# chao1224/MoleculeSDE

Hardware: AMD Instinct MI355X
Metric: molecules/sec pretrain step (SchNet+SDE VE, bs256) (higher is better)
Workload: dtype f32; 1 GPU; PCQM4Mv2-shaped pretrain step: GIN5x300 + SchNet(6x128f,51g,rc10) + EBM_node_dot_prod contrastive + SDEModel2Dto3D_02 VE; fwd+bwd+Adam; molecules_per_gpu=256, global_batch=256, parallelism=dp1

## Files before the change

### include/msde_hip.h

```cpp
#ifndef MSDE_HIP_H
#define MSDE_HIP_H

#ifdef __cplusplus
extern "C" {
#endif

#define MSDE_EINVAL (-1)
#define MSDE_EUNSUP (-2)

int msde_abi_version(void);
const char* msde_target_arch(void);

int msde_radius_count(const float* pos, const int* batch, const int* mol_ptr, int N, float r2,
                      int max_nbr, int* deg, void* stream);
int msde_exclusive_scan_i32(const int* in, int* out, int n, void* stream);
int msde_radius_fill(const float* pos, const int* batch, const int* mol_ptr, int N, float r2,
                     int max_nbr, const int* rowptr, int* src, int* dst, float* dist, int E_cap,
                     void* stream);


int msde_plan_build(const int* x_raw, int K, const int* atom_off, const int* bond_src, const int* bond_dst,
                    const int* bond_attr, const int* bond_off, const int* mol_atoms, const int* mol_bonds,
                    int B, int N_cap, int Eb_cap, int Ee_cap, int P_cap, int Er_cap, int max_nbr, int* mol_ptr,
                    int* bond_ptr, int* pair_ptr, int* sizes, int* batch_i32, int* atom_codes, int* z_codes, int* b_rowptr,
// ... 29 lines not shown
int msde_dd_transpose3(const float* x, int E, int to_soa, float* y, void* stream);
int msde_dd_merge3(const float* a, const float* b, const float* c, int E, float* y, void* stream);
int msde_dd_broadcast_rows(const float* b, int M, int K, float* y, void* stream);

int msde_combine_losses(const float* a, const float* b, const float* c, const float* d, float ca, float cb, float cc,
                        float cd, float* out, void* stream);
int msde_combine_losses_bwd(const float* g, float ca, float cb, float cc, float cd, float* out4, void* stream);
int msde_combine_losses_ex(const float* a, const float* b, const float* c, const float* d, float ca, float cb, float cc,
                           float cd, float* out, float* seeds4, const float* const* log_src, float* const* log_dst,
                           int n_log, void* stream);

int msde_debug_stamp(long long* slot, void* stream);

int msde_segment_sum_rows(const float* rows, int ldi ,
                          const int* rowptr, const int* perm, int N, int D,
                          float scale_by_inv_count, float* out, int ldo ,
                          void* stream);
int msde_segment_sum_rows2(const float* rows, int ldi, const int* rowptr, const int* perm, const int* rowptr2,
                           const int* perm2, int N, int D, float scale_by_inv_count, float* out, int ldo,
                           void* stream);
int msde_pair_gather_add(const float* A, const float* B, int ld, const int* src, const int* dst, int E,
                         int D, float* out, void* stream);
int msde_pair_gather_add_stats(const float* A, const float* B, int ld, const int* src, const int* dst, int E, int D,
                               const int* e_valid, float* out, float* stats, void* stream);
int msde_segment_sum_rows_bn(const float* G, const float* Z, int ld, const int* rowptr, const int* perm, int N, int D,
                             const float* p, const float* w, const float* u, float* out, int ldo, void* stream);
int msde_pair_strip(void);
int msde_pair_bn_dgrad_stats(const float* g, int ldg, const float* W, const float* Z, const float* scale, const float* shift,
                             const float* mean, int E, int H, int D, const int* e_valid, float* GA, float* stats,
                             void* stream);
int msde_pair_bn_scatter(const float* GA, const float* AB, int D, const int* src, const int* dst, const int* rowptr_s,
                         const int* perm_s, const int* rowptr, int N, const float* p, const float* w, const float* u,
                         float* gAB, void* stream);
int msde_pair_gather_cat(const float* X, int ldx, const float* C, int ldc, const int* src, const int* dst, int E,
                         int D, int D2, float* out, void* stream);
int msde_gather_rows(const float* X, const int* idx, int E, int D, float* out, void* stream);

int msde_radius_transpose(const int* batch, const int* mol_ptr, const int* rowptr, const int* src, int N,
                          int E_cap, int* deg_s, int* rowptr_s, int* perm_s, void* stream);
int msde_radius_transpose_mol(const int* mol_ptr, int B, int n_max, const int* rowptr, const int* src, int N, int E_cap,
                              int* rowptr_s, int* perm_s, void* stream);

int msde_embedding_sum_fwd(const float* tab, const int* codes, int N, int K, int D, float* out,
                           void* stream);
long long msde_embedding_sum_bwd_workspace_floats(int R, int D, int split);
int msde_embedding_sum_bwd(const float* g, const int* list_ptr, const int* list_nodes, int R,
                           int D, int split, float* g_tab, float* workspace, void* stream);

int msde_gin_aggregate_fwd(const float* x, const float* tab, const int* codes, const float* eps,
                           const int* rowptr, const int* src, int N, int D, float* out,
                           void* stream);
int msde_gin_aggregate_bwd_x(const float* g, const float* x, const float* tab, const int* codes,
                             const float* eps, const int* rowptr_s, const int* perm_s,
                             const int* dst, int N, int D, float* g_x, void* stream);
long long msde_gin_aggregate_bwd_tab_workspace_floats(int N, int E, int D, int R);
int msde_gin_aggregate_bn_fwd(const float* z, const float* scale, const float* shift, int relu, const float* tab,
                              const int* codes, const float* eps, const int* rowptr, const int* src, int N, int D,
                              float* h_out, float* out, void* stream);
int msde_gin_aggregate_bwd_x_stats(const float* g, const float* x, const float* tab, const int* codes, const float* eps,
                                   const int* rowptr_s, const int* perm_s, const int* dst, int N, const int* m_valid,
                                   int D, const float* zprev, const float* mean, int relu, float* g_x, float* stats,
                                   void* stream);
int msde_gin_aggregate_bwd_tab_slabs(int N, int E);
int msde_gin_aggregate_bwd_tab(const float* g, const float* x, const float* tab, const int* codes,
                               const int* src, const int* dst, int N, int E, int D, int R,
                               float* g_tab, float* g_eps, float* workspace, const int* n_dev, const int* e_dev,
// ... 440 lines not shown
```

### moleculesde_amd/_lib.py

```python
import ctypes
import os

_HERE = os.path.dirname(os.path.abspath(__file__))
LIB_PATH = os.path.join(_HERE, "csrc", "libmsde_hip.so")

P = ctypes.c_void_p
I = ctypes.c_int
F = ctypes.c_float
LL = ctypes.c_longlong
ULL = ctypes.c_ulonglong

SIGNATURES = {
    "msde_abi_version": [],
    "msde_target_arch": [],
    "msde_radius_count": [P, P, P, I, F, I, P, P],
    "msde_exclusive_scan_i32": [P, P, I, P],
    "msde_radius_fill": [P, P, P, I, F, I, P, P, P, P, I, P],
    "msde_segment_sum_rows": [P, I, P, P, I, I, F, P, I, P],
    "msde_segment_sum_rows2": [P, I, P, P, P, P, I, I, F, P, I, P],
    "msde_pair_gather_add": [P, P, I, P, P, I, I, P, P],
    "msde_pair_gather_add_stats": [P, P, I, P, P, I, I, P, P, P, P],
    "msde_segment_sum_rows_bn": [P, P, I, P, P, I, I, P, P, P, P, I, P],
    "msde_pair_strip": [],
    "msde_pair_bn_dgrad_stats": [P, I, P, P, P, P, P, I, I, I, P, P, P, P],
    "msde_pair_bn_scatter": [P, P, I, P, P, P, P, P, I, P, P, P, P, P],
    "msde_pair_gather_cat": [P, I, P, I, P, P, I, I, I, P, P],
    "msde_mlp_head_fwd": [P, I, P, P, I, I, I, P, P],
    "msde_mlp_head_bwd_slabs": [I, I],
    "msde_mlp_head_bwd": [P, I, P, P, I, I, I, P, P, P, P, P],
    "msde_mlp_head_mix_fwd": [P, I, P, P, I, P, P, I, P, P, P, P],
    "msde_mlp_head_mix_bwd": [P, I, P, P, P, P, P, I, I, P, P, P, P],
    "msde_gather_rows": [P, P, I, I, P, P],
    "msde_embedding_sum_fwd": [P, P, I, I, I, P, P],
    "msde_radius_transpose": [P, P, P, P, I, I, P, P, P, P],
    "msde_radius_transpose_mol": [P, I, I, P, P, I, I, P, P, P],
    "msde_embedding_sum_bwd_workspace_floats": [I, I, I],
    "msde_embedding_sum_bwd": [P, P, P, I, I, I, P, P, P],
    "msde_gin_aggregate_fwd": [P, P, P, P, P, P, I, I, P, P],
    "msde_gin_aggregate_bwd_x": [P, P, P, P, P, P, P, P, I, I, P, P],
    "msde_gin_aggregate_bn_fwd": [P, P, P, I, P, P, P, P, P, I, I, P, P, P],
    "msde_gin_aggregate_bwd_x_stats": [P, P, P, P, P, P, P, P, I, P, I, P, P, I, P, P, P],
    "msde_gin_aggregate_bwd_tab_workspace_floats": [I, I, I, I],
    "msde_gin_aggregate_bwd_tab": [P, P, P, P, P, P, I, I, I, I, P, P, P, P, P, P],
    "msde_gin_aggregate_bwd_tab_multi": [P, P, P, P, I, P, P, P, I, I, I, I, P, P, P],
    "msde_rbf_cutoff_fwd": [P, P, I, I, P, F, F, P, P, P],
    "msde_cfconv_aggregate_fwd": [P, P, P, P, P, I, I, P, P],
    "msde_cfconv_aggregate_bwd_w": [P, P, P, P, P, I, I, I, P, P],
    "msde_cfconv_aggregate_bwd_x": [P, P, P, P, P, P, I, I, P, P],
    "msde_cfconv_fused_fwd": [P, P, P, P, P, P, P, P, P, P, I, I, I, I, F, F, I, P, P, P],
    "msde_cfconv_fused_bwd_w_workspace_floats": [I, I, I],
    "msde_cfconv_fused_bwd_w_slabs": [I, I],
    "msde_gin_aggregate_bwd_tab_slabs": [I, I],
    "msde_cfconv_fused_bwd_w": [P, P, P, P, P, P, P, P, P, P, I, I, I, I, F, F, I, P, P, P, P, P, P],
    "msde_pair_build": [P, P, I, F, P, P, P, P, I, P, P],
    "msde_cfconv_pair_filter": [P, P, P, P, P, P, P, I, I, I, F, F, I, P, P],
    "msde_cfconv_pair_filter_multi": [P, P, P, P, P, P, P, I, I, I, I, F, F, I, P, P],
    "msde_cfconv_pair_bwd_w_multi_slabs": [I, I, I],
    "msde_cfconv_pair_bwd_w_multi": [P, P, P, P, P, P, P, P, P, P, I, I, I, I, I, F, F, I, P, P],
# ... 221 lines not shown
```

### moleculesde_amd/build.py

```python
import os
import subprocess
import sys
from concurrent.futures import ThreadPoolExecutor

HERE = os.path.dirname(os.path.abspath(__file__))
CSRC = os.path.join(HERE, "csrc")
OBJ = os.path.join(CSRC, "build")
LIB = os.path.join(CSRC, "libmsde_hip.so")
SOURCES = ["graph.hip", "gin.hip", "schnet.hip", "cfconv_fused.hip", "cfconv_fused_bwd.hip", "cfconv_pair.hip",
           "sde2d3d.hip", "linear.hip", "gemm_ex.hip", "gemm_rs.hip", "gemm_t2.hip", "gemm_t2_a1.hip", "gemm_t2_a2.hip", "dense_head.hip", "dense_pc.hip", "plan.hip", "dd.hip", "norm.hip",
           "contrastive.hip", "contrastive_infonce.hip", "optim.hip", "pointwise.hip", "gat_tail.hip", "escore_mol.hip", "escore_mol_bwd.hip",
           "molnet_head.hip", "qm9_head.hip", "md17.hip", "dataset.hip"]
HEADERS = [os.path.join(CSRC, "msde_common.h"), os.path.join(CSRC, "gemm_rs.h"), os.path.join(CSRC, "gemm_rs_epi.h"), os.path.join(CSRC, "gemm_t2.h"), os.path.join(CSRC, "escore_mol.h"),
           os.path.join(HERE, "..", "include", "msde_hip.h")]


def _flags():
    return ["--offload-arch=gfx950", "-O3", "-std=c++17", "-fPIC", "-Wno-unused-result", "-Wno-unused-value"] + \
        os.environ.get("MSDE_HIPCC_FLAGS", "").split()


def _stale(target, deps):
    if not os.path.exists(target):
        return True
    t = os.path.getmtime(target)
    return any(os.path.exists(d) and os.path.getmtime(d) > t for d in deps)


def needs_build():
    srcs = [os.path.join(CSRC, s) for s in SOURCES if os.path.exists(os.path.join(CSRC, s))]
    return _stale(LIB, srcs + HEADERS)


def build(force=False, verbose=True):
    if not force and not needs_build():
        return LIB
    hipcc = os.environ.get("HIPCC", "/opt/rocm/bin/hipcc")
    os.makedirs(OBJ, exist_ok=True)
    flags = _flags()
    stamp = os.path.join(OBJ, "flags.txt")
    old = open(stamp).read() if os.path.exists(stamp) else None
    if old != " ".join(flags):
        force = True
    jobs, objs = [], []
    for s in SOURCES:
# ... 26 lines not shown
```

### moleculesde_amd/csrc/graph.hip

```cpp
#include "msde_common.h"

__global__ void radius_count_kernel(const float* __restrict__ pos, const int* __restrict__ batch,
                                    const int* __restrict__ mol_ptr, int N, float r2, int max_nbr,
                                    int* __restrict__ deg) {
  int i = blockIdx.x * blockDim.x + threadIdx.x;
  if (i >= N) return;
  int m = batch[i];
  int j0 = mol_ptr[m], j1 = mol_ptr[m + 1];
  float xi = pos[3 * i], yi = pos[3 * i + 1], zi = pos[3 * i + 2];
  int cnt = 0;
  for (int j = j0; j < j1 && cnt < max_nbr; ++j) {
    if (j == i) continue;
    float dx = xi - pos[3 * j], dy = yi - pos[3 * j + 1], dz = zi - pos[3 * j + 2];
    float d2 = dx * dx + dy * dy + dz * dz;
    cnt += (d2 < r2) ? 1 : 0;
  }
  deg[i] = cnt;
}

__global__ void radius_fill_kernel(const float* __restrict__ pos, const int* __restrict__ batch,
                                   const int* __restrict__ mol_ptr, int N, float r2, int max_nbr,
                                   const int* __restrict__ rowptr, int* __restrict__ src,
                                   int* __restrict__ dst, float* __restrict__ dist, int E_cap) {
  int i = blockIdx.x * blockDim.x + threadIdx.x;
// ... 290 lines not shown
    return;
  }
  const T* a = reinterpret_cast<const T*>(A) + (size_t)j * ld_cols;
  if (B) {
    const T* b = reinterpret_cast<const T*>(B) + (size_t)i * ld_cols;
    for (int c = lane; c < cols; c += tpr) O[c] = vadd(a[c], b[c]);
  } else {
    for (int c = lane; c < cols; c += tpr) O[c] = a[c];
  }
}

extern "C" int msde_pair_gather_add(const float* A, const float* B, int ld, const int* src, const int* dst, int E,
                                    int D, float* out, void* stream) {
  if (E < 0 || D <= 0 || !A || !B || !src || !dst || !out) return MSDE_EINVAL;
  if (ld == 0) ld = D;
  if (ld < D) return MSDE_EINVAL;
  if (E == 0) return 0;
  const bool vec = D % 4 == 0 && ld % 4 == 0 &&
                   ((reinterpret_cast<uintptr_t>(A) | reinterpret_cast<uintptr_t>(B) | reinterpret_cast<uintptr_t>(out)) & 15) == 0;
  if (vec) {
    int cols = D / 4, tpr = pick_tpr(cols), rpb = 256 / tpr;
    MSDE_LAUNCH(pair_gather_add_kernel<4>, dim3((E + rpb - 1) / rpb), dim3(256), 0, as_stream(stream), A, B,
                       src, dst, E, cols, ld / 4, tpr, out);
  } else {
    int cols = D, tpr = pick_tpr(cols), rpb = 256 / tpr;
    MSDE_LAUNCH(pair_gather_add_kernel<1>, dim3((E + rpb - 1) / rpb), dim3(256), 0, as_stream(stream), A, B,
                       src, dst, E, cols, ld, tpr, out);
  }
  MSDE_CHECK_LAUNCH();
  return 0;
}

#define MSDE_PAIR_STRIP 128
__global__ void __launch_bounds__(512)
pair_gather_add_stats_kernel(const float4* __restrict__ A, const float4* __restrict__ B, int ld4, const int* __restrict__ src,
                             const int* __restrict__ dst, int E, const int* __restrict__ e_valid, int CL, int SR,
                             float4* __restrict__ out, float* __restrict__ stats) {
  __shared__ float4 p1[512], p2[512];
  const int RL = 512 / CL;
  const int cl = threadIdx.x % CL, rl = threadIdx.x / CL;
  const int e0 = blockIdx.x * SR;
  const int ev = e_valid ? min(E, e_valid[0]) : E;
  const bool active = rl < RL;
  float4 sh = make_float4(0.f, 0.f, 0.f, 0.f), s1 = sh, s2 = sh;
  if (active && e0 < ev) {
    const int j = src[e0], i = dst[e0];
    if (j >= 0) sh = vadd(A[(size_t)j * ld4 + cl], B[(size_t)i * ld4 + cl]);
  }
  if (active) {
    for (int r = rl; r < SR; r += 4 * RL) {
      float4 v[4];
      int e[4];
#pragma unroll
      for (int k = 0; k < 4; ++k) {
        e[k] = e0 + r + k * RL;
        const bool in = (r + k * RL < SR) && e[k] < E;
        const int j = in ? src[e[k]] : -1, i = in ? dst[e[k]] : 0;
        v[k] = j >= 0 ? vadd(A[(size_t)j * ld4 + cl], B[(size_t)i * ld4 + cl]) : make_float4(0.f, 0.f, 0.f, 0.f);
        if (!in) e[k] = -1;
      }
#pragma unroll
      for (int k = 0; k < 4; ++k) {
        if (e[k] < 0) continue;
        out[(size_t)e[k] * CL + cl] = v[k];
        if (e[k] < ev) {
          const float4 d = make_float4(v[k].x - sh.x, v[k].y - sh.y, v[k].z - sh.z, v[k].w - sh.w);
          s1 = vadd(s1, d);
          s2.x = fmaf(d.x, d.x, s2.x); s2.y = fmaf(d.y, d.y, s2.y); s2.z = fmaf(d.z, d.z, s2.z); s2.w = fmaf(d.w, d.w, s2.w);
        }
      }
    }
  }
  p1[threadIdx.x] = s1;
  p2[threadIdx.x] = s2;
  __syncthreads();
  if (rl == 0) {
    for (int q = 1; q < RL; ++q) { s1 = vadd(s1, p1[q * CL + cl]); s2 = vadd(s2, p2[q * CL + cl]); }
    const int n = max(0, min(SR, ev - e0));
    const float inv = n > 0 ? 1.f / (float)n : 0.f;
    float4 mean, m2;
    mean.x = sh.x + s1.x * inv; mean.y = sh.y + s1.y * inv; mean.z = sh.z + s1.z * inv; mean.w = sh.w + s1.w * inv;
    m2.x = fmaxf(s2.x - s1.x * s1.x * inv, 0.f); m2.y = fmaxf(s2.y - s1.y * s1.y * inv, 0.f);
    m2.z = fmaxf(s2.z - s1.z * s1.z * inv, 0.f); m2.w = fmaxf(s2.w - s1.w * s1.w * inv, 0.f);
    float4* st = reinterpret_cast<float4*>(stats + (size_t)blockIdx.x * 2 * (4 * CL));
    st[cl] = mean;
    st[CL + cl] = m2;
  }
}

extern "C" int msde_pair_gather_add_stats(const float* A, const float* B, int ld, const int* src, const int* dst, int E,
                                          int D, const int* e_valid, float* out, float* stats, void* stream) {
  if (E < 0 || D <= 0 || !A || !B || !src || !dst || !out || !stats) return MSDE_EINVAL;
  if (ld == 0) ld = D;
  if (ld < D) return MSDE_EINVAL;
  if (D % 4 || ld % 4 || D > 1024 ||
      ((reinterpret_cast<uintptr_t>(A) | reinterpret_cast<uintptr_t>(B) | reinterpret_cast<uintptr_t>(out) |
        reinterpret_cast<uintptr_t>(stats)) & 15))
    return MSDE_EUNSUP;
  if (E == 0) return 0;
  MSDE_LAUNCH(pair_gather_add_stats_kernel, dim3((E + MSDE_PAIR_STRIP - 1) / MSDE_PAIR_STRIP), dim3(512), 0, as_stream(stream),
              reinterpret_cast<const float4*>(A), reinterpret_cast<const float4*>(B), ld / 4, src, dst, E, e_valid, D / 4,
              MSDE_PAIR_STRIP, reinterpret_cast<float4*>(out), stats);
  MSDE_CHECK_LAUNCH();
  return 0;
}

template <int H>
__device__ __forceinline__ float4 pbd_row(const float* __restrict__ gr_, const float4 (&w)[H]) {
  const float4* gr = reinterpret_cast<const float4*>(gr_);
  float4 a = make_float4(0.f, 0.f, 0.f, 0.f);
#pragma unroll
  for (int q = 0; q < H / 4; ++q) {
    const float4 gv = gr[q];
    a.x = fmaf(gv.x, w[4 * q].x, a.x); a.y = fmaf(gv.x, w[4 * q].y, a.y); a.z = fmaf(gv.x, w[4 * q].z, a.z); a.w = fmaf(gv.x, w[4 * q].w, a.w);
    a.x = fmaf(gv.y, w[4 * q + 1].x, a.x); a.y = fmaf(gv.y, w[4 * q + 1].y, a.y); a.z = fmaf(gv.y, w[4 * q + 1].z, a.z); a.w = fmaf(gv.y, w[4 * q + 1].w, a.w);
    a.x = fmaf(gv.z, w[4 * q + 2].x, a.x); a.y = fmaf(gv.z, w[4 * q + 2].y, a.y); a.z = fmaf(gv.z, w[4 * q + 2].z, a.z); a.w = fmaf(gv.z, w[4 * q + 2].w, a.w);
    a.x = fmaf(gv.w, w[4 * q + 3].x, a.x); a.y = fmaf(gv.w, w[4 * q + 3].y, a.y); a.z = fmaf(gv.w, w[4 * q + 3].z, a.z); a.w = fmaf(gv.w, w[4 * q + 3].w, a.w);
  }
  return a;
}

template <int H>
__global__ void __launch_bounds__(512)
pair_bn_dgrad_stats_kernel(const float* __restrict__ g, int ldg, const float4* __restrict__ W, const float4* __restrict__ Z,
                           const float4* __restrict__ scale, const float4* __restrict__ shift, const float4* __restrict__ mean,
                           int E, const int* __restrict__ e_valid, int CL, int SR, float4* __restrict__ GA,
                           float* __restrict__ stats) {
  extern __shared__ __attribute__((aligned(16))) float gs[];
  __shared__ float4 p1[512], p2[512];
  const int RL = 512 / CL;
  const int cl = threadIdx.x % CL, rl = threadIdx.x / CL;
  const int e0 = blockIdx.x * SR;
  const int ev = e_valid ? min(E, e_valid[0]) : E;
  const bool active = rl < RL;
  for (int t = threadIdx.x; t < SR * (H / 4); t += 512) {
    const int r = t / (H / 4), q = t - r * (H / 4);
    const int e = e0 + r;
    reinterpret_cast<float4*>(gs)[t] = e < E ? *reinterpret_cast<const float4*>(g + (size_t)e * ldg + 4 * q)
                                             : make_float4(0.f, 0.f, 0.f, 0.f);
  }
  float4 w[H];
  float4 sc = make_float4(0.f, 0.f, 0.f, 0.f), sf = sc, mu = sc;
  if (active) {
#pragma unroll
    for (int h = 0; h < H; ++h) w[h] = W[(size_t)h * CL + cl];
    sc = scale[cl]; sf = shift[cl]; mu = mean[cl];
  }
  __syncthreads();
  float4 s1 = make_float4(0.f, 0.f, 0.f, 0.f), s2 = s1;
  auto finish = [&](int e, float4 a, const float4& z) __attribute__((always_inline)) {
    a.x = fmaf(z.x, sc.x, sf.x) > 0.f ? a.x : 0.f;
    a.y = fmaf(z.y, sc.y, sf.y) > 0.f ? a.y : 0.f;
    a.z = fmaf(z.z, sc.z, sf.z) > 0.f ? a.z : 0.f;
    a.w = fmaf(z.w, sc.w, sf.w) > 0.f ? a.w : 0.f;
    GA[(size_t)e * CL + cl] = a;
    if (e < ev) {
      s1 = vadd(s1, a);
      s2.x = fmaf(a.x, z.x - mu.x, s2.x); s2.y = fmaf(a.y, z.y - mu.y, s2.y);
      s2.z = fmaf(a.z, z.z - mu.z, s2.z); s2.w = fmaf(a.w, z.w - mu.w, s2.w);
    }
  };
  if (active) {
    const int nrows = min(SR, E - e0);
    for (int r = rl; r < nrows; r += 4 * RL) {
      float4 z[4];
#pragma unroll
      for (int k = 0; k < 4; ++k) {
        const int rr = r + k * RL;
        z[k] = rr < nrows ? Z[(size_t)(e0 + rr) * CL + cl] : make_float4(0.f, 0.f, 0.f, 0.f);
      }
#pragma unroll
      for (int k = 0; k < 4; ++k) {
        const int rr = r + k * RL;
        if (rr < nrows) finish(e0 + rr, pbd_row<H>(gs + rr * H, w), z[k]);
      }
    }
  }
  p1[threadIdx.x] = s1;
  p2[threadIdx.x] = s2;
  __syncthreads();
  if (rl == 0) {
    for (int q = 1; q < RL; ++q) { s1 = vadd(s1, p1[q * CL + cl]); s2 = vadd(s2, p2[q * CL + cl]); }
    float4* st = reinterpret_cast<float4*>(stats + (size_t)blockIdx.x * 2 * (4 * CL));
    st[cl] = s1;
    st[CL + cl] = s2;
  }
}

extern "C" int msde_pair_bn_dgrad_stats(const float* g, int ldg, const float* W, const float* Z, const float* scale,
                                        const float* shift, const float* mean, int E, int H, int D, const int* e_valid,
                                        float* GA, float* stats, void* stream) {
  if (E < 0 || H <= 0 || D <= 0 || !g || !W || !Z || !scale || !shift || !mean || !GA || !stats) return MSDE_EINVAL;
  if (ldg <= 0) ldg = H;
  if ((H != 16 && H != 32) || D % 4 || D > 1024 || ldg % 4 ||
      ((reinterpret_cast<uintptr_t>(g) | reinterpret_cast<uintptr_t>(W) | reinterpret_cast<uintptr_t>(Z) |
        reinterpret_cast<uintptr_t>(scale) | reinterpret_cast<uintptr_t>(shift) | reinterpret_cast<uintptr_t>(mean) |
        reinterpret_cast<uintptr_t>(GA) | reinterpret_cast<uintptr_t>(stats)) & 15))
    return MSDE_EUNSUP;
  if (E == 0) return 0;
  const dim3 grid((E + MSDE_PAIR_STRIP - 1) / MSDE_PAIR_STRIP);
  const size_t lds = (size_t)MSDE_PAIR_STRIP * H * sizeof(float);
#define PBD_GO(H_) MSDE_LAUNCH(pair_bn_dgrad_stats_kernel<H_>, grid, dim3(512), lds, as_stream(stream), g, ldg,                     \
                               reinterpret_cast<const float4*>(W), reinterpret_cast<const float4*>(Z),                             \
                               reinterpret_cast<const float4*>(scale), reinterpret_cast<const float4*>(shift),                    \
                               reinterpret_cast<const float4*>(mean), E, e_valid, D / 4, MSDE_PAIR_STRIP,                          \
                               reinterpret_cast<float4*>(GA), stats)
  if (H == 16) PBD_GO(16); else PBD_GO(32);
#undef PBD_GO
  MSDE_CHECK_LAUNCH();
  return 0;
}

__global__ void __launch_bounds__(256)
pair_bn_scatter_kernel(const float4* __restrict__ GA, const float4* __restrict__ AB, int ldab4,
                       const int* __restrict__ src, const int* __restrict__ dst,
                       const int* __restrict__ rowptr_s, const int* __restrict__ perm_s,
                       const int* __restrict__ rowptr, int N, int cols, const float4* __restrict__ p,
                       const float4* __restrict__ w, const float4* __restrict__ u, float4* __restrict__ out, int ldo4) {
  const int rpb = 256 / cols;
  const int c = threadIdx.x % cols, rw = threadIdx.x / cols;
  const int row = blockIdx.x * rpb + rw;
  if (rw >= rpb || row >= 2 * N) return;
  const bool by_src = row < N;
  const int i = by_src ? row : row - N;
  const int* rp = by_src ? rowptr_s : rowptr;
  const int s0 = rp[i], s1 = rp[i + 1];
  const float cnt = (float)(s1 - s0);
  const float4* other = AB + (by_src ? cols : 0);
  const int* oidx = by_src ? dst : src;
  float4 ag = make_float4(0.f, 0.f, 0.f, 0.f), az = ag;
  int s = s0;
  for (; s + 3 < s1; s += 4) {
    int e[4];
#pragma unroll
    for (int k = 0; k < 4; ++k) e[k] = by_src ? perm_s[s + k] : s + k;
    float4 gv[4], zv[4];
#pragma unroll
    for (int k = 0; k < 4; ++k) {
      gv[k] = GA[(size_t)e[k] * cols + c];
      zv[k] = other[(size_t)oidx[e[k]] * ldab4 + c];
    }
    ag = vadd(vadd(vadd(vadd(ag, gv[0]), gv[1]), gv[2]), gv[3]);
    az = vadd(vadd(vadd(vadd(az, zv[0]), zv[1]), zv[2]), zv[3]);
// ... 334 lines not shown
```

### moleculesde_amd/hip.py

```python
import ctypes

import weakref as _weakref

import torch

from . import _lib


from ._torchabi import _stream, _p, _f32, _i32


import contextlib as _contextlib

_BOUNDS = {}


@_contextlib.contextmanager
def row_bounds(bounds):
    global _BOUNDS
    for t in bounds.values():
        assert t.dtype == torch.int32 and t.is_cuda and t.numel() >= 1
    prev, _BOUNDS = _BOUNDS, {int(c): t for c, t in bounds.items()}
    try:
        yield
# ... 2092 lines not shown
                      act="relu", dact_from=a1, stats=sta, stats_mode="bnbwd", stats_z=z1, stats_mean=v1[2])
        if not fused_fin:
            pw1, gb1 = _bn_fin_bwd(sta, sa, M, H, g1, v1[2], v1[3])
        dz1 = torch.empty(M, H, dtype=torch.float32, device=dev)
        g_agg = torch.empty(M, D, dtype=torch.float32, device=dev) if ctx.needs_input_grad[0] else None
        if BN_BWD_PASS:
            if fused_fin:
                gb1 = _bn_bwd_fin_cols(sta, sa, M, H, g1, v1[2], v1[3], ga1, z1, None, None, dz1, rows)
            else:
                _lib.call("msde_bn_bwd_cols", _p(ga1), _ld(ga1), _p(z1), _ld(z1), _p(pw1[0]), _p(pw1[1]), _p(pw1[2]), _p(None), _p(None),
                          M, _p(rows), H, _p(dz1), H, st)
            if g_agg is not None:
                gemm_node(dz1, W1, g_agg, False, D, H)
        elif g_agg is not None:
            gemm_node(ga1, W1, g_agg, False, D, H, axf="bnbwd", xf=(pw1[0], pw1[1], pw1[2]), A2=z1, A_out=dz1)
        else:
            scratch = torch.empty(M, D, dtype=torch.float32, device=dev)
            gemm_node(ga1, W1, scratch, False, D, H, axf="bnbwd", xf=(pw1[0], pw1[1], pw1[2]), A2=z1, A_out=dz1)
        gW2, gbias2 = weight_grad(dz2, a1, True, ctx.deferrable)
        gW1, gbias1 = weight_grad(dz1, agg, True, ctx.deferrable)
        return (g_agg, gW1, gbias1, gb1[0], gb1[1], None, None, gW2, gbias2, gb2[0], gb2[1], None, None,
                None, None, None, None, None, None)


def gin_mlp_bn(agg, lin1, bn1, lin2, bn2, relu_out, defer_apply=False):
    box = [] if defer_apply else None
    h = _GinMlpBN.apply(agg, lin1.weight, lin1.bias, bn1.weight, bn1.bias, bn1.running_mean, bn1.running_var,
                        lin2.weight, lin2.bias, bn2.weight, bn2.bias, bn2.running_mean, bn2.running_var,
                        bn1.eps, 0.1 if bn1.momentum is None else bn1.momentum, bn2.eps,
                        0.1 if bn2.momentum is None else bn2.momentum, relu_out, box)
    return (h, box[0]) if defer_apply else h


class _PairBnReluLinear(torch.autograd.Function):

    @staticmethod
    def forward(ctx, AB, plan, gamma, beta, rm, rv, eps, momentum, W2, b2):
        AB = _f32(AB)
        E, D = plan.E, AB.size(1) // 2
        H = W2.size(0)
        dev = AB.device
        SR = pair_strip()
        strips = (E + SR - 1) // SR
        pre = torch.empty(E, D, dtype=torch.float32, device=dev)
        st = torch.empty(strips, 2, D, dtype=torch.float32, device=dev)
        _lib.call("msde_pair_gather_add_stats", _p(AB), AB.data_ptr() + 4 * D, 2 * D, _p(plan.src), _p(plan.dst), E, D,
                  _p(bound_tensor(E)), _p(pre), _p(st), _stream())
        v = _bn_fin_fwd(st, strips, SR, E, D, gamma, beta, eps, momentum, rm, rv)
        y = torch.empty(E, D, dtype=torch.float32, device=dev)
        out = torch.empty(E, H, dtype=torch.float32, device=dev)
        gemm_node(pre, W2, out, True, H, D, bias=b2, axf="affine", xf=(v[0], v[1]), relu=True, A_out=y)
        ctx.save_for_backward(pre, y, v, W2, gamma, AB)
        ctx.plan = plan
        ctx.deferrable = all(t.is_leaf or getattr(t, "_msde_leaf_like", False) for t in (W2, b2))
        return out

    @staticmethod
    def backward(ctx, g):
        pre, y, v, W2, gamma, AB = ctx.saved_tensors
        plan = ctx.plan
        g = _f32(g)
        E, D = pre.shape
        H = W2.size(0)
        dev = g.device
        ga = torch.empty(E, D, dtype=torch.float32, device=dev)
        if H in (16, 32) and W2.is_contiguous() and W2.data_ptr() % 16 == 0:
            SR = pair_strip()
            sa = (E + SR - 1) // SR
            sta = torch.empty(sa, 2, D, dtype=torch.float32, device=dev)
            _lib.call("msde_pair_bn_dgrad_stats", _p(g), _ld(g), _p(W2), _p(pre), _p(v[0]), _p(v[1]), _p(v[2]), E, H, D,
                      _p(bound_tensor(E)), _p(ga), _p(sta), _stream())
        else:
            sa, _ = rs_geometry(E, D, H)
            sta = torch.empty(sa, 2, D, dtype=torch.float32, device=dev)
            gemm_node(g, W2, ga, False, D, H, act="relu", dact_from=y, stats=sta, stats_mode="bnbwd", stats_z=pre,
                      stats_mean=v[2])
        pw, gb = _bn_fin_bwd(sta, sa, E, D, gamma, v[2], v[3])
        g_AB = None
        if ctx.needs_input_grad[0]:
            g_AB = torch.empty(plan.N, 2 * D, dtype=torch.float32, device=dev)
            _lib.call("msde_pair_bn_scatter", _p(ga), _p(AB), D, _p(plan.src), _p(plan.dst), _p(plan.rowptr_s), _p(plan.perm_s),
                      _p(plan.rowptr), plan.N, _p(pw[0]), _p(pw[1]), _p(pw[2]), _p(g_AB), _stream())
        gW2, gb2 = weight_grad(g, y, True, ctx.deferrable)
        return g_AB, None, gb[0], gb[1], None, None, None, None, gW2, gb2


_PAIR_STRIP = None


def pair_strip():
    global _PAIR_STRIP
    if _PAIR_STRIP is None:
        _PAIR_STRIP = int(_lib.load().msde_pair_strip())
    return _PAIR_STRIP


def pair_bn_relu_linear_ok(AB, bn, lin2):
    D = AB.size(1) // 2
    return (AB.is_cuda and AB.dtype == torch.float32 and AB.dim() == 2 and AB.size(1) == 2 * D and D % 4 == 0 and D <= 768
# ... 73 lines not shown
```

Baseline: 105,400 molecules/s.

## Fuse pair gather-add into BN-ReLU-linear to avoid materializing pre-activation tensor

Adds a pair_emb forward kernel that gathers A[src]+B[dst] on the fly, applies the BN affine and ReLU, writes y, and runs the small H=16/32 projection with MFMA, so the E×D pre-activation tensor is never stored. The stats kernel gets a no-store variant and stages src/dst indices in shared memory. Backward gains a gather variant of the BN dgrad/stats kernel that recomputes the pre-activation from A/B instead of reading a saved copy. This cuts E×D write and read traffic and memory footprint, at the cost of extra random gathers, one more gather pass in the forward, and a new large-LDS kernel.

After: 106,100 molecules/s (median of 6 runs). About the same (+0.7%).

```diff
diff --git a/include/msde_hip.h b/include/msde_hip.h
--- a/include/msde_hip.h
+++ b/include/msde_hip.h
@@ -85,6 +85,12 @@
 int msde_pair_bn_scatter(const float* GA, const float* AB, int D, const int* src, const int* dst, const int* rowptr_s,
                          const int* perm_s, const int* rowptr, int N, const float* p, const float* w, const float* u,
                          float* gAB, void* stream);
+int msde_pair_emb_fwd(const float* A, const float* B, int ld, const int* src, const int* dst, int E, int D, int H,
+                      const float* W2, const float* bias, const float* scale, const float* shift, float* y, float* out,
+                      void* stream);
+int msde_pair_bn_dgrad_stats_ab(const float* g, int ldg, const float* W, const float* A, const float* B, int ld,
+                                const int* src, const int* dst, const float* scale, const float* shift, const float* mean,
+                                int E, int H, int D, const int* n_edges, float* GA, float* stats, void* stream);
 int msde_pair_gather_cat(const float* X, int ldx, const float* C, int ldc, const int* src, const int* dst, int E,
                          int D, int D2, float* out, void* stream);
 int msde_gather_rows(const float* X, const int* idx, int E, int D, float* out, void* stream);
diff --git a/moleculesde_amd/_lib.py b/moleculesde_amd/_lib.py
--- a/moleculesde_amd/_lib.py
+++ b/moleculesde_amd/_lib.py
@@ -24,6 +24,8 @@
     "msde_pair_strip": [],
     "msde_pair_bn_dgrad_stats": [P, I, P, P, P, P, P, I, I, I, P, P, P, P],
     "msde_pair_bn_scatter": [P, P, I, P, P, P, P, P, I, P, P, P, P, P],
+    "msde_pair_emb_fwd": [P, P, I, P, P, I, I, I, P, P, P, P, P, P, P],
+    "msde_pair_bn_dgrad_stats_ab": [P, I, P, P, P, I, P, P, P, P, P, I, I, I, P, P, P, P],
     "msde_pair_gather_cat": [P, I, P, I, P, P, I, I, I, P, P],
     "msde_mlp_head_fwd": [P, I, P, P, I, I, I, P, P],
     "msde_mlp_head_bwd_slabs": [I, I],
diff --git a/moleculesde_amd/build.py b/moleculesde_amd/build.py
--- a/moleculesde_amd/build.py
+++ b/moleculesde_amd/build.py
@@ -10,7 +10,7 @@
 SOURCES = ["graph.hip", "gin.hip", "schnet.hip", "cfconv_fused.hip", "cfconv_fused_bwd.hip", "cfconv_pair.hip",
            "sde2d3d.hip", "linear.hip", "gemm_ex.hip", "gemm_rs.hip", "gemm_t2.hip", "gemm_t2_a1.hip", "gemm_t2_a2.hip", "dense_head.hip", "dense_pc.hip", "plan.hip", "dd.hip", "norm.hip",
            "contrastive.hip", "contrastive_infonce.hip", "optim.hip", "pointwise.hip", "gat_tail.hip", "escore_mol.hip", "escore_mol_bwd.hip",
-           "molnet_head.hip", "qm9_head.hip", "md17.hip", "dataset.hip"]
+           "molnet_head.hip", "qm9_head.hip", "md17.hip", "dataset.hip", "pair_emb.hip"]
 HEADERS = [os.path.join(CSRC, "msde_common.h"), os.path.join(CSRC, "gemm_rs.h"), os.path.join(CSRC, "gemm_rs_epi.h"), os.path.join(CSRC, "gemm_t2.h"), os.path.join(CSRC, "escore_mol.h"),
            os.path.join(HERE, "..", "include", "msde_hip.h")]
 
diff --git a/moleculesde_amd/csrc/graph.hip b/moleculesde_amd/csrc/graph.hip
--- a/moleculesde_amd/csrc/graph.hip
+++ b/moleculesde_amd/csrc/graph.hip
@@ -346,19 +346,28 @@
 }
 
 #define MSDE_PAIR_STRIP 128
+template <bool STORE>
 __global__ void __launch_bounds__(512)
 pair_gather_add_stats_kernel(const float4* __restrict__ A, const float4* __restrict__ B, int ld4, const int* __restrict__ src,
                              const int* __restrict__ dst, int E, const int* __restrict__ e_valid, int CL, int SR,
                              float4* __restrict__ out, float* __restrict__ stats) {
   __shared__ float4 p1[512], p2[512];
+  __shared__ int si[MSDE_PAIR_STRIP], di[MSDE_PAIR_STRIP];
   const int RL = 512 / CL;
   const int cl = threadIdx.x % CL, rl = threadIdx.x / CL;
-  const int e0 = blockIdx.x * SR;
+  const int strip = blockIdx.x;
+  const int e0 = strip * SR;
   const int ev = e_valid ? min(E, e_valid[0]) : E;
   const bool active = rl < RL;
+  if (threadIdx.x < SR) {
+    const int e = e0 + threadIdx.x;
+    si[threadIdx.x] = e < E ? src[e] : -1;
+    di[threadIdx.x] = e < E ? dst[e] : 0;
+  }
+  __syncthreads();
   float4 sh = make_float4(0.f, 0.f, 0.f, 0.f), s1 = sh, s2 = sh;
   if (active && e0 < ev) {
-    const int j = src[e0], i = dst[e0];
+    const int j = si[0], i = di[0];
     if (j >= 0) sh = vadd(A[(size_t)j * ld4 + cl], B[(size_t)i * ld4 + cl]);
   }
   if (active) {
@@ -369,14 +378,14 @@
       for (int k = 0; k < 4; ++k) {
         e[k] = e0 + r + k * RL;
         const bool in = (r + k * RL < SR) && e[k] < E;
-        const int j = in ? src[e[k]] : -1, i = in ? dst[e[k]] : 0;
+        const int j = in ? si[r + k * RL] : -1, i = in ? di[r + k * RL] : 0;
         v[k] = j >= 0 ? vadd(A[(size_t)j * ld4 + cl], B[(size_t)i * ld4 + cl]) : make_float4(0.f, 0.f, 0.f, 0.f);
         if (!in) e[k] = -1;
       }
 #pragma unroll
       for (int k = 0; k < 4; ++k) {
         if (e[k] < 0) continue;
-        out[(size_t)e[k] * CL + cl] = v[k];
+        if (STORE) out[(size_t)e[k] * CL + cl] = v[k];
         if (e[k] < ev) {
           const float4 d = make_float4(v[k].x - sh.x, v[k].y - sh.y, v[k].z - sh.z, v[k].w - sh.w);
           s1 = vadd(s1, d);
@@ -396,7 +405,7 @@
     mean.x = sh.x + s1.x * inv; mean.y = sh.y + s1.y * inv; mean.z = sh.z + s1.z * inv; mean.w = sh.w + s1.w * inv;
     m2.x = fmaxf(s2.x - s1.x * s1.x * inv, 0.f); m2.y = fmaxf(s2.y - s1.y * s1.y * inv, 0.f);
     m2.z = fmaxf(s2.z - s1.z * s1.z * inv, 0.f); m2.w = fmaxf(s2.w - s1.w * s1.w * inv, 0.f);
-    float4* st = reinterpret_cast<float4*>(stats + (size_t)blockIdx.x * 2 * (4 * CL));
+    float4* st = reinterpret_cast<float4*>(stats + (size_t)strip * 2 * (4 * CL));
     st[cl] = mean;
     st[CL + cl] = m2;
   }
@@ -404,7 +413,7 @@
 
 extern "C" int msde_pair_gather_add_stats(const float* A, const float* B, int ld, const int* src, const int* dst, int E,
                                           int D, const int* e_valid, float* out, float* stats, void* stream) {
-  if (E < 0 || D <= 0 || !A || !B || !src || !dst || !out || !stats) return MSDE_EINVAL;
+  if (E < 0 || D <= 0 || !A || !B || !src || !dst || !stats) return MSDE_EINVAL;
   if (ld == 0) ld = D;
   if (ld < D) return MSDE_EINVAL;
   if (D % 4 || ld % 4 || D > 1024 ||
@@ -412,9 +421,12 @@
         reinterpret_cast<uintptr_t>(stats)) & 15))
     return MSDE_EUNSUP;
   if (E == 0) return 0;
-  MSDE_LAUNCH(pair_gather_add_stats_kernel, dim3((E + MSDE_PAIR_STRIP - 1) / MSDE_PAIR_STRIP), dim3(512), 0, as_stream(stream),
-              reinterpret_cast<const float4*>(A), reinterpret_cast<const float4*>(B), ld / 4, src, dst, E, e_valid, D / 4,
-              MSDE_PAIR_STRIP, reinterpret_cast<float4*>(out), stats);
+#define PGS_GO(STORE_) MSDE_LAUNCH(pair_gather_add_stats_kernel<STORE_>, dim3((E + MSDE_PAIR_STRIP - 1) / MSDE_PAIR_STRIP),        \
+                                  dim3(512), 0, as_stream(stream), reinterpret_cast<const float4*>(A),                            \
+                                  reinterpret_cast<const float4*>(B), ld / 4, src, dst, E, e_valid, D / 4, MSDE_PAIR_STRIP,        \
+                                  reinterpret_cast<float4*>(out), stats)
+  if (out) PGS_GO(true); else PGS_GO(false);
+#undef PGS_GO
   MSDE_CHECK_LAUNCH();
   return 0;
 }
@@ -434,17 +446,21 @@
   return a;
 }
 
-template <int H>
+template <int H, bool GATHER>
 __global__ void __launch_bounds__(512)
 pair_bn_dgrad_stats_kernel(const float* __restrict__ g, int ldg, const float4* __restrict__ W, const float4* __restrict__ Z,
-                           const float4* __restrict__ scale, const float4* __restrict__ shift, const float4* __restrict__ mean,
+                           const float4* __restrict__ A, const float4* __restrict__ B, int ld4,
+                           const int* __restrict__ src, const int* __restrict__ dst, const float4* __restrict__ scale,
+                           const float4* __restrict__ shift, const float4* __restrict__ mean,
                            int E, const int* __restrict__ e_valid, int CL, int SR, float4* __restrict__ GA,
                            float* __restrict__ stats) {
   extern __shared__ __attribute__((aligned(16))) float gs[];
   __shared__ float4 p1[512], p2[512];
+  __shared__ int si[GATHER ? MSDE_PAIR_STRIP : 1], di[GATHER ? MSDE_PAIR_STRIP : 1];
   const int RL = 512 / CL;
   const int cl = threadIdx.x % CL, rl = threadIdx.x / CL;
-  const int e0 = blockIdx.x * SR;
+  const int strip = blockIdx.x;
+  const int e0 = strip * SR;
   const int ev = e_valid ? min(E, e_valid[0]) : E;
   const bool active = rl < RL;
   for (int t = threadIdx.x; t < SR * (H / 4); t += 512) {
@@ -452,6 +468,11 @@
     const int e = e0 + r;
     reinterpret_cast<float4*>(gs)[t] = e < E ? *reinterpret_cast<const float4*>(g + (size_t)e * ldg + 4 * q)
                                              : make_float4(0.f, 0.f, 0.f, 0.f);
+  }
+  if (GATHER && threadIdx.x < SR) {
+    const int e = e0 + threadIdx.x;
+    si[threadIdx.x] = e < E ? src[e] : -1;
+    di[threadIdx.x] = e < E ? dst[e] : 0;
   }
   float4 w[H];
   float4 sc = make_float4(0.f, 0.f, 0.f, 0.f), sf = sc, mu = sc;
@@ -474,7 +495,37 @@
       s2.z = fmaf(a.z, z.z - mu.z, s2.z); s2.w = fmaf(a.w, z.w - mu.w, s2.w);
     }
   };
-  if (active) {
+  if (GATHER) {
+    if (active) {
+      const int nrows = min(SR, E - e0);
+      float4 za[4], zb[4];
+      auto request = [&](int r) __attribute__((always_inline)) {
+#pragma unroll
+        for (int k = 0; k < 4; ++k) {
+          const int rc = min(r + k * RL, SR - 1);
+          za[k] = A[(size_t)max(si[rc], 0) * ld4 + cl];
+          zb[k] = B[(size_t)max(di[rc], 0) * ld4 + cl];
+        }
+      };
+      request(rl);
+      for (int r = rl; r < nrows; r += 4 * RL) {
+        float4 z[4];
+#pragma unroll
+        for (int k = 0; k < 4; ++k) {
+          const int rr = r + k * RL;
+          const bool live = rr < nrows && si[min(rr, SR - 1)] >= 0;
+          const float4 t = vadd(za[k], zb[k]);
+          z[k] = make_float4(live ? t.x : 0.f, live ? t.y : 0.f, live ? t.z : 0.f, live ? t.w : 0.f);
+        }
+        request(r + 4 * RL);
+#pragma unroll
+        for (int k = 0; k < 4; ++k) {
+          const int rr = r + k * RL;
+          if (rr < nrows) finish(e0 + rr, pbd_row<H>(gs + rr * H, w), z[k]);
+        }
+      }
+    }
+  } else if (active) {
     const int nrows = min(SR, E - e0);
     for (int r = rl; r < nrows; r += 4 * RL) {
       float4 z[4];
@@ -495,34 +546,57 @@
   __syncthreads();
   if (rl == 0) {
     for (int q = 1; q < RL; ++q) { s1 = vadd(s1, p1[q * CL + cl]); s2 = vadd(s2, p2[q * CL + cl]); }
-    float4* st = reinterpret_cast<float4*>(stats + (size_t)blockIdx.x * 2 * (4 * CL));
+    float4* st = reinterpret_cast<float4*>(stats + (size_t)strip * 2 * (4 * CL));
     st[cl] = s1;
     st[CL + cl] = s2;
   }
 }
 
-extern "C" int msde_pair_bn_dgrad_stats(const float* g, int ldg, const float* W, const float* Z, const float* scale,
-                                        const float* shift, const float* mean, int E, int H, int D, const int* e_valid,
-                                        float* GA, float* stats, void* stream) {
-  if (E < 0 || H <= 0 || D <= 0 || !g || !W || !Z || !scale || !shift || !mean || !GA || !stats) return MSDE_EINVAL;
+static int pair_bn_dgrad_launch(const float* g, int ldg, const float* W, const float* Z, const float* A, const float* B, int ld,
+                                const int* src, const int* dst, const float* scale, const float* shift, const float* mean,
+                                int E, int H, int D, const int* e_valid, float* GA, float* stats, void* stream) {
+  const bool gather = Z == nullptr;
+  if (E < 0 || H <= 0 || D <= 0 || !g || !W || !scale || !shift || !mean || !GA || !stats) return MSDE_EINVAL;
+  if (gather ? (!A || !B || !src || !dst) : false) return MSDE_EINVAL;
   if (ldg <= 0) ldg = H;
-  if ((H != 16 && H != 32) || D % 4 || D > 1024 || ldg % 4 ||
+  if (ld == 0) ld = D;
+  if (gather && ld < D) return MSDE_EINVAL;
+  if ((H != 16 && H != 32) || D % 4 || D > 1024 || ldg % 4 || (gather && ld % 4) ||
       ((reinterpret_cast<uintptr_t>(g) | reinterpret_cast<uintptr_t>(W) | reinterpret_cast<uintptr_t>(Z) |
+        reinterpret_cast<uintptr_t>(A) | reinterpret_cast<uintptr_t>(B) |
         reinterpret_cast<uintptr_t>(scale) | reinterpret_cast<uintptr_t>(shift) | reinterpret_cast<uintptr_t>(mean) |
         reinterpret_cast<uintptr_t>(GA) | reinterpret_cast<uintptr_t>(stats)) & 15))
     return MSDE_EUNSUP;
   if (E == 0) return 0;
   const dim3 grid((E + MSDE_PAIR_STRIP - 1) / MSDE_PAIR_STRIP);
   const size_t lds = (size_t)MSDE_PAIR_STRIP * H * sizeof(float);
-#define PBD_GO(H_) MSDE_LAUNCH(pair_bn_dgrad_stats_kernel<H_>, grid, dim3(512), lds, as_stream(stream), g, ldg,                     \
-                               reinterpret_cast<const float4*>(W), reinterpret_cast<const float4*>(Z),                             \
-                               reinterpret_cast<const float4*>(scale), reinterpret_cast<const float4*>(shift),                    \
-                               reinterpret_cast<const float4*>(mean), E, e_valid, D / 4, MSDE_PAIR_STRIP,                          \
-                               reinterpret_cast<float4*>(GA), stats)
-  if (H == 16) PBD_GO(16); else PBD_GO(32);
+#define PBD_GO(H_, G_) MSDE_LAUNCH((pair_bn_dgrad_stats_kernel<H_, G_>), grid, dim3(512), lds, as_stream(stream), g, ldg,          \
+                                   reinterpret_cast<const float4*>(W), reinterpret_cast<const float4*>(Z),                         \
+                                   reinterpret_cast<const float4*>(A), reinterpret_cast<const float4*>(B), ld / 4, src, dst,       \
+                                   reinterpret_cast<const float4*>(scale), reinterpret_cast<const float4*>(shift),                \
+                                   reinterpret_cast<const float4*>(mean), E, e_valid, D / 4, MSDE_PAIR_STRIP,                      \
+                                   reinterpret_cast<float4*>(GA), stats)
+  if (gather) { if (H == 16) PBD_GO(16, true); else PBD_GO(32, true); }
+  else { if (H == 16) PBD_GO(16, false); else PBD_GO(32, false); }
 #undef PBD_GO
   MSDE_CHECK_LAUNCH();
   return 0;
+}
+
+extern "C" int msde_pair_bn_dgrad_stats(const float* g, int ldg, const float* W, const float* Z, const float* scale,
+                                        const float* shift, const float* mean, int E, int H, int D, const int* e_valid,
+                                        float* GA, float* stats, void* stream) {
+  if (!Z) return MSDE_EINVAL;
+  return pair_bn_dgrad_launch(g, ldg, W, Z, nullptr, nullptr, 0, nullptr, nullptr, scale, shift, mean, E, H, D, e_valid, GA,
+                              stats, stream);
+}
+
+extern "C" int msde_pair_bn_dgrad_stats_ab(const float* g, int ldg, const float* W, const float* A, const float* B, int ld,
+                                           const int* src, const int* dst, const float* scale, const float* shift,
+                                           const float* mean, int E, int H, int D, const int* n_edges, float* GA,
+                                           float* stats, void* stream) {
+  if (!A || !B || !src || !dst) return MSDE_EINVAL;
+  return pair_bn_dgrad_launch(g, ldg, W, nullptr, A, B, ld, src, dst, scale, shift, mean, E, H, D, n_edges, GA, stats, stream);
 }
 
 __global__ void __launch_bounds__(256)
diff --git a/moleculesde_amd/csrc/pair_emb.hip b/moleculesde_amd/csrc/pair_emb.hip
--- /dev/null
+++ b/moleculesde_amd/csrc/pair_emb.hip
@@ -0,0 +1,161 @@
+#include "gemm_rs.h"
+#include <map>
+#include <mutex>
+
+#define PE_WAVES 8
+#define PE_SB 5
+#define PE_TB 2
+
+template <int RN>
+__global__ void __launch_bounds__(64 * PE_WAVES)
+pair_emb_fwd_kernel(const float4* __restrict__ A, const float4* __restrict__ B, int ld4, const int* __restrict__ src,
+                    const int* __restrict__ dst, int E, int D, const float4* __restrict__ W2, const float* __restrict__ bias,
+                    const float4* __restrict__ scale, const float4* __restrict__ shift, float4* __restrict__ y,
+                    float* __restrict__ out) {
+  extern __shared__ __attribute__((aligned(16))) float4 pe_smem[];
+  const int nt = (D + 31) >> 5, D4 = D >> 2, KP4 = 8 * nt;
+  float4* __restrict__ Wf = pe_smem;
+  float4* __restrict__ sc = Wf + (size_t)2 * nt * RN * 64;
+  float4* __restrict__ sf = sc + KP4;
+  const int wave = threadIdx.x >> 6, lane = threadIdx.x & 63, r = lane & 15, q = lane >> 4;
+  const int tile0 = blockIdx.x * (16 * PE_WAVES) + 16 * wave;
+  const int e = tile0 + r;
+  int j = -1, i = 0;
+  if (e < E) { j = src[e]; i = dst[e]; }
+  const bool live = j >= 0;
+  const float4* __restrict__ pa = A + (size_t)(live ? j : 0) * ld4;
+  const float4* __restrict__ pb = B + (size_t)(live ? i : 0) * ld4;
+  auto load = [&](int t0, float4 (&xa)[2 * PE_TB], float4 (&xb)[2 * PE_TB]) __attribute__((always_inline)) {
+#pragma unroll
+    for (int u = 0; u < 2 * PE_TB; ++u) {
+      const int k4 = 8 * t0 + 4 * u + q;
+      xa[u] = pa[min(k4, D4 - 1)];
+      xb[u] = pb[min(k4, D4 - 1)];
+    }
+  };
+  float4 ca[2 * PE_TB], cb[2 * PE_TB], na[2 * PE_TB], nb[2 * PE_TB];
+  load(0, ca, cb);
+  for (int base = threadIdx.x; base < 2 * nt * RN * 64; base += PE_SB * 64 * PE_WAVES) {
+    float4 w[PE_SB];
+#pragma unroll
+    for (int v = 0; v < PE_SB; ++v) {
+      const int idx = base + v * 64 * PE_WAVES;
+      const int l = idx & 63, c = (idx >> 6) % RN, s = idx / (64 * RN);
+      const int k4 = 4 * s + (l >> 4);
+      const int row = RN * (l & 15) + c;
+      w[v] = W2[(size_t)row * D4 + min(k4, D4 - 1)];
+      if (k4 >= D4) w[v] = make_float4(0.f, 0.f, 0.f, 0.f);
+    }
+#pragma unroll
+    for (int v = 0; v < PE_SB; ++v) {
+      const int idx = base + v * 64 * PE_WAVES;
+      if (idx < 2 * nt * RN * 64) Wf[idx] = w[v];
+    }
+  }
+  for (int k4 = threadIdx.x; k4 < KP4; k4 += 64 * PE_WAVES) {
+    float4 a = make_float4(0.f, 0.f, 0.f, 0.f), b = a;
+    if (k4 < D4) { a = scale[k4]; b = shift[k4]; }
+    sc[k4] = a;
+    sf[k4] = b;
+  }
+  __syncthreads();
+  f32x4 acc[2][RN];
+#pragma unroll
+  for (int h = 0; h < 2; ++h)
+#pragma unroll
+    for (int c = 0; c < RN; ++c) acc[h][c] = f32x4{0.f, 0.f, 0.f, 0.f};
+  const bool skip_last = D - (nt - 1) * 32 <= 16;
+  const int nbatch = (nt + PE_TB - 1) / PE_TB;
+  auto compute = [&](int b, const float4 (&xa)[2 * PE_TB], const float4 (&xb)[2 * PE_TB]) __attribute__((always_inline)) {
+#pragma unroll
+    for (int u = 0; u < 2 * PE_TB; ++u) {
+      const int t = b * PE_TB + (u >> 1), h = u & 1, s = 2 * t + h;
+      if (t < nt) {
+        const int k4 = 4 * s + q;
+        const bool ok = live && k4 < D4;
+        float4 x = vadd(xa[u], xb[u]);
+        x.x = ok ? x.x : 0.f; x.y = ok ? x.y : 0.f; x.z = ok ? x.z : 0.f; x.w = ok ? x.w : 0.f;
+        const float4 scv = sc[k4], sfv = sf[k4];
+        float4 a;
+        a.x = fmaxf(fmaf(x.x, scv.x, sfv.x), 0.f); a.y = fmaxf(fmaf(x.y, scv.y, sfv.y), 0.f);
+        a.z = fmaxf(fmaf(x.z, scv.z, sfv.z), 0.f); a.w = fmaxf(fmaf(x.w, scv.w, sfv.w), 0.f);
+        if (e < E && k4 < D4) y[(size_t)e * D4 + k4] = a;
+        if (!(h == 1 && t == nt - 1 && skip_last)) {
+          float4 bf[RN];
+#pragma unroll
+          for (int c = 0; c < RN; ++c) bf[c] = Wf[(size_t)(s * RN + c) * 64 + lane];
+#pragma unroll
+          for (int jj = 0; jj < 4; ++jj)
+#pragma unroll
+            for (int c = 0; c < RN; ++c) acc[h][c] = rs_mfma(rs_f4(a, jj), rs_f4(bf[c], jj), acc[h][c]);
+        }
+      }
+    }
+  };
+  for (int b = 0; b < nbatch; b += 2) {
+    load((b + 1) * PE_TB, na, nb);
+    compute(b, ca, cb);
+    load((b + 2) * PE_TB, ca, cb);
+    compute(b + 1, na, nb);
+  }
+  const int n = lane & 15, H = 16 * RN;
+  float bv[RN];
+#pragma unroll
+  for (int c = 0; c < RN; ++c) bv[c] = bias ? bias[RN * n + c] : 0.f;
+#pragma unroll
+  for (int el = 0; el < 4; ++el) {
+    const int row = tile0 + 4 * q + el;
+    if (row >= E) continue;
+    float v[RN];
+#pragma unroll
+    for (int c = 0; c < RN; ++c) v[c] = acc[0][c][el] + (acc[1][c][el] + bv[c]);
+    float* o = out + (size_t)row * H + RN * n;
+    if (RN == 2) *reinterpret_cast<float2*>(o) = make_float2(v[0], v[RN - 1]);
+    else o[0] = v[0];
+  }
+}
+
+static size_t pe_lds_bytes(int rn, int D) {
+  const int nt = (D + 31) / 32;
+  return ((size_t)2 * nt * rn * 64 + (size_t)2 * 8 * nt) * sizeof(float4);
+}
+
+template <typename KERN, typename... ARGS>
+static int pe_launch(KERN kern, dim3 grid, size_t lds, hipStream_t st, ARGS... args) {
+  if (lds > 64 * 1024) {
+    static std::map<const void*, size_t> granted;
+    static std::mutex mu;
+    std::lock_guard<std::mutex> lk(mu);
+    size_t& gr = granted[reinterpret_cast<const void*>(kern)];
+    if (lds > gr) {
+      hipError_t err = hipFuncSetAttribute(reinterpret_cast<const void*>(kern), hipFuncAttributeMaxDynamicSharedMemorySize, (int)lds);
+      if (err != hipSuccess) return (int)err;
+      gr = lds;
+    }
+  }
+  MSDE_LAUNCH(kern, grid, dim3(64 * PE_WAVES), lds, st, args...);
+  MSDE_CHECK_LAUNCH();
+  return 0;
+}
+
+extern "C" int msde_pair_emb_fwd(const float* A, const float* B, int ld, const int* src, const int* dst, int E, int D, int H,
+                                 const float* W2, const float* bias, const float* scale, const float* shift, float* y,
+                                 float* out, void* stream) {
+  if (E < 0 || D <= 0 || H <= 0 || !A || !B || !src || !dst || !W2 || !scale || !shift || !y || !out) return MSDE_EINVAL;
+  if (ld == 0) ld = D;
+  if (ld < D) return MSDE_EINVAL;
+  if ((H != 16 && H != 32) || D % 4 || ld % 4 || D > 768 ||
+      ((reinterpret_cast<uintptr_t>(A) | reinterpret_cast<uintptr_t>(B) | reinterpret_cast<uintptr_t>(W2) |
+        reinterpret_cast<uintptr_t>(scale) | reinterpret_cast<uintptr_t>(shift) | reinterpret_cast<uintptr_t>(y) |
+        reinterpret_cast<uintptr_t>(out)) & 15))
+    return MSDE_EUNSUP;
+  if (E == 0) return 0;
+  const dim3 grid((E + 16 * PE_WAVES - 1) / (16 * PE_WAVES));
+  const size_t lds = pe_lds_bytes(H / 16, D);
+#define PE_GO(RN_) pe_launch(pair_emb_fwd_kernel<RN_>, grid, lds, as_stream(stream), reinterpret_cast<const float4*>(A),          \
+                             reinterpret_cast<const float4*>(B), ld / 4, src, dst, E, D, reinterpret_cast<const float4*>(W2),     \
+                             bias, reinterpret_cast<const float4*>(scale), reinterpret_cast<const float4*>(shift),              \
+                             reinterpret_cast<float4*>(y), out)
+  return H == 16 ? PE_GO(1) : PE_GO(2);
+#undef PE_GO
+}
diff --git a/moleculesde_amd/hip.py b/moleculesde_amd/hip.py
--- a/moleculesde_amd/hip.py
+++ b/moleculesde_amd/hip.py
@@ -2148,6 +2148,14 @@
     return (h, box[0]) if defer_apply else h
 
 
+PAIR_EMB_NO_PRE = True
+
+
+def _pair_emb_no_pre_ok(E, D, H, W2):
+    return (PAIR_EMB_NO_PRE and H in (16, 32) and W2.is_contiguous() and W2.data_ptr() % 16 == 0 and D <= 768
+            and t2_ok(E, H, D, "bnbwd"))
+
+
 class _PairBnReluLinear(torch.autograd.Function):
 
     @staticmethod
@@ -2158,29 +2166,43 @@
         dev = AB.device
         SR = pair_strip()
         strips = (E + SR - 1) // SR
-        pre = torch.empty(E, D, dtype=torch.float32, device=dev)
+        no_pre = _pair_emb_no_pre_ok(E, D, H, W2)
+        pre = None if no_pre else torch.empty(E, D, dtype=torch.float32, device=dev)
         st = torch.empty(strips, 2, D, dtype=torch.float32, device=dev)
         _lib.call("msde_pair_gather_add_stats", _p(AB), AB.data_ptr() + 4 * D, 2 * D, _p(plan.src), _p(plan.dst), E, D,
                   _p(bound_tensor(E)), _p(pre), _p(st), _stream())
         v = _bn_fin_fwd(st, strips, SR, E, D, gamma, beta, eps, momentum, rm, rv)
         y = torch.empty(E, D, dtype=torch.float32, device=dev)
         out = torch.empty(E, H, dtype=torch.float32, device=dev)
-        gemm_node(pre, W2, out, True, H, D, bias=b2, axf="affine", xf=(v[0], v[1]), relu=True, A_out=y)
-        ctx.save_for_backward(pre, y, v, W2, gamma, AB)
+        if no_pre:
+            _lib.call("msde_pair_emb_fwd", _p(AB), AB.data_ptr() + 4 * D, 2 * D, _p(plan.src), _p(plan.dst), E, D, H, _p(W2),
+                      _p(b2), _p(v[0]), _p(v[1]), _p(y), _p(out), _stream())
+            ctx.save_for_backward(y, v, W2, gamma, AB)
+        else:
+            gemm_node(pre, W2, out, True, H, D, bias=b2, axf="affine", xf=(v[0], v[1]), relu=True, A_out=y)
+            ctx.save_for_backward(y, v, W2, gamma, AB, pre)
+        ctx.no_pre = no_pre
         ctx.plan = plan
         ctx.deferrable = all(t.is_leaf or getattr(t, "_msde_leaf_like", False) for t in (W2, b2))
         return out
 
     @staticmethod
     def backward(ctx, g):
-        pre, y, v, W2, gamma, AB = ctx.saved_tensors
+        y, v, W2, gamma, AB = ctx.saved_tensors[:5]
+        pre = None if ctx.no_pre else ctx.saved_tensors[5]
         plan = ctx.plan
         g = _f32(g)
-        E, D = pre.shape
+        E, D = y.shape
         H = W2.size(0)
         dev = g.device
         ga = torch.empty(E, D, dtype=torch.float32, device=dev)
-        if H in (16, 32) and W2.is_contiguous() and W2.data_ptr() % 16 == 0:
+        if ctx.no_pre:
+            SR = pair_strip()
+            sa = (E + SR - 1) // SR
+            sta = torch.empty(sa, 2, D, dtype=torch.float32, device=dev)
+            _lib.call("msde_pair_bn_dgrad_stats_ab", _p(g), _ld(g), _p(W2), _p(AB), AB.data_ptr() + 4 * D, 2 * D, _p(plan.src),
+                      _p(plan.dst), _p(v[0]), _p(v[1]), _p(v[2]), E, H, D, _p(bound_tensor(E)), _p(ga), _p(sta), _stream())
+        elif H in (16, 32) and W2.is_contiguous() and W2.data_ptr() % 16 == 0:
             SR = pair_strip()
             sa = (E + SR - 1) // SR
             sta = torch.empty(sa, 2, D, dtype=torch.float32, device=dev)
```
